# OpenMatchmaking/microservice-matchmaking

Hardware: AMD Instinct MI355X
Metric: matched players/sec over 1M-player pool (higher is better)
Workload: dtype int32

## Files before the change

include/mm_engine.h:

```cpp
#ifndef MM_ENGINE_H
#define MM_ENGINE_H

#include <stdint.h>

#ifdef __cplusplus
extern "C" {
#endif

#define MM_ABI_VERSION 1u

#define MM_MAX_GROUPS 16u
#define MM_MAX_MODES  16u
#define MM_MAX_ROLES  8u
#define MM_MAX_TEAMS  4u
#define MM_MAX_LOBBY  16u

#define MM_CONS_MODE(c)   ((uint32_t)(c) & 0xFu)
#define MM_CONS_REGION(c) (((uint32_t)(c) >> 4) & 0xFFu)
#define MM_CONS_PARTY(c)  (((uint32_t)(c) >> 12) & 0xFu)
#define MM_CONS_ROLE(c)   (((uint32_t)(c) >> 16) & 0xFu)
#define MM_CONS_MAKE(mode, region, party, role)                                          \
    (((uint32_t)(mode) & 0xFu) | (((uint32_t)(region) & 0xFFu) << 4) |                  \
     (((uint32_t)(party) & 0xFu) << 12) | (((uint32_t)(role) & 0xFu) << 16))
#define MM_CONS_USER_MASK 0x000FFFFFu
// ... 93 lines not shown
    uint32_t pair_ptimeout_us;
    uint32_t pair_pinject;
    uint32_t pair_tiles_max;
    uint32_t pair_tile_fixed;
    uint32_t pair_xcd;
    uint32_t pair_group_min;
    uint32_t pair_nxseg;
    uint32_t pair_nxstage;
    uint32_t pair_tune;
    uint32_t team_batch;
    uint32_t team_f2;
    uint32_t team_rebuild;
    uint32_t team_emit_max;
    uint32_t team_split;
    uint32_t team_fwait;
    uint32_t team_fix_max;
    uint32_t team_fix_t8;
    uint32_t team_fix_t4;
    uint32_t team_pull_xcd;
    uint32_t team_nowait;
    uint32_t team_late;
    uint32_t team_late0;
    uint32_t team_cap;
} mm_tuning;

int mm_tuning_default(mm_tuning* t);
int mm_tuning_set(mm_tuning* t, const char* name, uint32_t value);
const char* mm_tuning_name(uint32_t index);
int mm_engine_create_ex(const mm_config* cfg, const mm_tuning* tuning, mm_engine** out);
int mm_tuning_get(const mm_engine* e, mm_tuning* t);

int mm_reset(mm_engine* e);


int mm_enqueue(mm_engine* e, uint32_t n, const int32_t* rating, const uint32_t* cons,
               const uint8_t* group, uint32_t* out_slot, mm_enqueue_stats* st);

int mm_enqueue_device(mm_engine* e, uint32_t n, const int32_t* d_rating,
                      const uint32_t* d_cons, uint32_t* first_slot, mm_enqueue_stats* st);

int mm_cancel(mm_engine* e, uint32_t n, const uint32_t* slot);


int mm_tick(mm_engine* e, uint32_t mode, uint32_t* n_matches, mm_stats* stats);

int mm_matches(mm_engine* e, uint32_t first, uint32_t count, uint32_t* slots, float* score,
// ... 42 lines not shown
    uint32_t crit_round_passes;
    uint32_t crit_late_passes;
    uint32_t crit_late_lobbies;
    uint32_t degraded;
    uint32_t crit_timed_passes;
    uint32_t crit_timed_hops;
    uint32_t crit_barrier_cycles;
    uint32_t crit_hop_cycles;
    uint32_t clk_cycles;
    uint32_t clk_wall_ticks;
    uint32_t pair_nx_init_ns;
    uint32_t pair_tested_lo, pair_tested_hi;
    uint32_t pair_tested_nx_lo, pair_tested_nx_hi;
    uint32_t crit_team_group;
    uint32_t crit_team_passes;
    uint32_t crit_team_f_passes;
    uint32_t crit_team_fc_passes;
    uint32_t crit_team_late_passes;
    uint32_t crit_team_f_lobbies;
    uint32_t crit_team_fc_lobbies;
    uint32_t crit_team_late_lobbies;
    uint32_t crit_team_lookups;
    uint32_t crit_team_late_lookups;
} mm_path_stats;
int mm_path_stats_get(mm_engine* e, mm_path_stats* out);

int mm_last_hip_error(const mm_engine* e);

#ifdef __cplusplus
}
#endif
#endif
```

microservice_matchmaking_amd/_abi.py:

```python
from __future__ import annotations

import ctypes as C
import time
from dataclasses import dataclass

import numpy as np

MM_ABI_VERSION = 1
MM_MAX_GROUPS = 16
MM_MAX_MODES = 16
MM_MAX_ROLES = 8
MM_MAX_TEAMS = 4
MM_MAX_LOBBY = 16
MM_MODE_REGION_FILTER = 1
MM_MODE_PARTY_FILTER = 2
MM_CFG_TIMING = 1
MM_WAIT_HIST = 33
NO_SLOT = 0xFFFFFFFF

STATUS_NAMES = {
    0: "MM_OK", -1: "MM_ERR_INVALID_ARG", -2: "MM_ERR_NO_DEVICE", -3: "MM_ERR_OOM",
    -4: "MM_ERR_FULL", -5: "MM_ERR_HIP", -6: "MM_ERR_INTERNAL", -7: "MM_ERR_ABI",
    -8: "MM_ERR_RANGE", -9: "MM_ERR_STATE",
}
# ... 34 lines not shown


class MMEnqueueStats(C.Structure):
    _fields_ = [("accepted", C.c_uint32), ("rejected", C.c_uint32),
                ("bucket_ms", C.c_float), ("total_ms", C.c_float)]

    def as_dict(self):
        return {n: getattr(self, n) for n, _ in self._fields_}


class MMPathStats(C.Structure):
    _fields_ = [(n, C.c_uint32) for n in (
        "size", "mode", "paths", "host_looks",
        "pair_rounds_launches", "pair_rounds_passes", "pair_round_launches", "pair_tiled_passes",
        "pair_stops_timeout", "pair_stops_xcd", "pair_stops_inject", "pair_yields",
        "pair_persist_off", "pair_cooldown", "pair_stops_total",
        "team_f_launches", "team_fc_launches", "team_late_launches", "team_build_launches",
        "team_flags_late", "team_flags_late_total",
        "crit_group", "crit_passes", "crit_rounds_passes", "crit_rounds_hops", "crit_round_passes", "crit_late_passes",
        "crit_late_lobbies", "degraded",
        "crit_timed_passes", "crit_timed_hops", "crit_barrier_cycles", "crit_hop_cycles", "clk_cycles", "clk_wall_ticks",
        "pair_nx_init_ns", "pair_tested_lo", "pair_tested_hi", "pair_tested_nx_lo", "pair_tested_nx_hi",
        "crit_team_group", "crit_team_passes", "crit_team_f_passes", "crit_team_fc_passes", "crit_team_late_passes",
        "crit_team_f_lobbies", "crit_team_fc_lobbies", "crit_team_late_lobbies", "crit_team_lookups", "crit_team_late_lookups")]

    def as_dict(self):
        return {n: int(getattr(self, n)) for n, _ in self._fields_ if n != "size"}


class MMWaitGroup(C.Structure):
    _fields_ = [("waiting", C.c_uint32), ("oldest_age", C.c_uint32), ("age_sum", C.c_uint64),
                ("hist", C.c_uint32 * MM_WAIT_HIST), ("pad", C.c_uint32)]

    def as_dict(self):
        return {"waiting": int(self.waiting), "oldest_age": int(self.oldest_age), "age_sum": int(self.age_sum),
                "hist": np.asarray(self.hist[:], dtype=np.uint32)}


class MMError(RuntimeError):
    def __init__(self, status, where):
        self.status = int(status)
        super().__init__("%s failed: %s (%d)" % (where, STATUS_NAMES.get(self.status, "?"), self.status))


def cons_make(mode=0, region=0, party=0, role=0):
    mode, region, party, role = (np.asarray(x, dtype=np.uint32) for x in (mode, region, party, role))
    return ((mode & 0xF) | ((region & 0xFF) << 4) | ((party & 0xF) << 12) | ((role & 0xF) << 16)).astype(np.uint32)
# ... 416 lines not shown
```

microservice_matchmaking_amd/csrc/mm_engine.hip:

```cpp
#include <hip/hip_runtime.h>

#include <stdint.h>
#include <stdio.h>
#include <stdlib.h>
#include <string.h>
#include <time.h>

#include <dlfcn.h>

#include <algorithm>
#include <mutex>
#include <cmath>
#include <new>
#include <vector>

#include "../../include/mm_engine.h"
#include "../../include/mm_wait.h"
#include <mm_gfx950.h>


#define MM_NO_SLOT 0xFFFFFFFFu
#define MM_ST_FREE 0
#define MM_ST_LIVE 1
#define MM_ST_CANCELLED 2
// ... 904 lines not shown
    uint32_t* d_tk_chunkB;
    uint32_t* d_tk_fdone;
    uint32_t team_seq;
    uint32_t* d_tk_sqi;
    uint32_t tk_memb;
    uint32_t tk_chunk_stride;
    std::vector<uint32_t> tk_last_len;
    uint32_t dbg_last_w, dbg_last_c;
    ChainDev* h_chains;
    uint32_t* h_counters;
    std::vector<uint8_t> h_state;
    uint32_t next_slot;
    uint32_t cancel_pending;
    std::vector<uint32_t> r_released;
    uint32_t* h_rslots;
    float* h_rscore;
    uint32_t* h_rpass;
    uint32_t r_n, r_L;
    hipStream_t copy_stream;
    hipEvent_t ev_copy;
    bool ev_copy_pending;
    uint32_t r_base[MM_MAX_GROUPS], r_cnt[MM_MAX_GROUPS], r_pre[MM_MAX_GROUPS + 1];
    uint32_t r_sent[MM_MAX_GROUPS];
    uint32_t r_marked[MM_MAX_GROUPS];
    bool r_based;
    bool poisoned;
    uint32_t ticks_seen;
    bool clock_on;
    uint32_t clock_now;
    uint32_t* d_stamp;
    uint32_t* d_wt_rows;
    uint32_t wt_max_chunks;
    uint32_t* d_wt_out;
    WaitGroupDev* d_wt_stats;
    uint32_t* d_wt_matched;
    std::vector<uint32_t> x_slot, x_group, x_age;
    std::vector<uint32_t> x_new;
    std::vector<int32_t> x_rating;
    std::vector<uint32_t> x_cons, x_stamp;
    uint32_t* d_mv_cols;
    uint8_t* d_mv_group;
    uint32_t* h_mwait;
    uint32_t mw_n;
};

struct RoctxApi {
// ... 293 lines not shown
    MM_TD(pair_ptimeout_us, "MM_PAIR_PTIMEOUT_US", 5000u, 0u, 1000000u, 0u),
    MM_TD(pair_pinject, "MM_PAIR_PINJECT", 0u, 0u, 0xFFFFFFFFu, 0u),
    MM_TD(pair_tiles_max, "MM_PAIR_TILES", PK_TILES_MAX, 1u, 4096u, 0u),
    MM_TD(pair_tile_fixed, "MM_PAIR_TILE", 0u, 0u, 1u, 0u),
    MM_TD(pair_xcd, "MM_PAIR_XCD", 1u, 0u, 1u, 0u),
    MM_TD(pair_group_min, "MM_PAIR_GROUP", PK_GROUP_MIN, 0u, 0xFFFFFFFFu, 0u),
    MM_TD(pair_nxseg, "MM_PAIR_NXSEG", 0u, 64u, NXI_SEG, 1u),
    MM_TD(pair_nxstage, "MM_PAIR_NXSTAGE", 0u, 0u, 0xFFFFFFFFu, 0u),
    MM_TD(pair_tune, "MM_PAIR_TUNE", 0u, 0u, 0xFFFFFFFFu, 0u),
    MM_TD(team_batch, "MM_TEAM_BATCH", 16u, 1u, 4096u, 0u),
    MM_TD(team_f2, "MM_TEAM_F2", 32u, 0u, 0xFFFFFFFFu, 0u),
    MM_TD(team_rebuild, "MM_TEAM_REBUILD", 8u, 1u, 4096u, 0u),
    MM_TD(team_emit_max, "MM_TEAM_EMIT_MAX", TC_EMIT_MAX, 1u, TC_EMIT_MAX, 0u),
    MM_TD(team_split, "MM_TEAM_SPLIT", 1u, 0u, 1u, 0u),
    MM_TD(team_fwait, "MM_TEAM_FWAIT", 1u << 14, 0u, 0xFFFFFFFFu, 0u),
    MM_TD(team_fix_max, "MM_TEAM_FIXMAX", 0xFFFFFFFFu, 0u, 0xFFFFFFFFu, 0u),
    MM_TD(team_fix_t8, "MM_TEAM_FIXT8", 10u, 0u, 0xFFFFFFFFu, 0u),
    MM_TD(team_fix_t4, "MM_TEAM_FIXT4", 64u, 0u, 0xFFFFFFFFu, 0u),
    MM_TD(team_pull_xcd, "MM_TEAM_PULLX", 1u, 0u, 1u, 0u),
    MM_TD(team_nowait, "MM_TEAM_NOWAIT", 0u, 0u, 0xFFFFFFFFu, 0u),
    MM_TD(team_late, "MM_TEAM_LATE", 6u, 0u, 0xFFFFFFFFu, 0u),
    MM_TD(team_late0, "MM_TEAM_LATE0", 512u, 0u, 0xFFFFFFFFu, 0u),
    MM_TD(team_cap, "MM_TEAM_CAP", TT_SCAN_CAP, 1u, 4096u, 0u),
};
#undef MM_TD
static const uint32_t k_tune_n = (uint32_t)(sizeof(k_tune) / sizeof(k_tune[0]));
static_assert(sizeof(mm_tuning) == (sizeof(k_tune) / sizeof(k_tune[0]) + 1u) * sizeof(uint32_t), "every field of mm_tuning has its row in k_tune");

static bool tune_in_range(const TuneDesc& d, uint32_t v)
{
    if (d.kind == 1u) return v == 0u || (v >= d.lo && v <= d.hi && (v & (v - 1u)) == 0u);
    return v >= d.lo && v <= d.hi;
}
static uint32_t& tune_field(mm_tuning* t, const TuneDesc& d) { return *(uint32_t*)((char*)t + d.off); }

static void tune_defaults(mm_tuning* full)
{
    full->size = (uint32_t)sizeof(mm_tuning);
    for (uint32_t i = 0; i < k_tune_n; ++i) {
        const TuneDesc& d = k_tune[i];
        uint32_t v = d.def;
        const char* s = getenv(d.env);
        if (s && *s) {
            char* end = NULL;
            unsigned long long x = strtoull(s, &end, 0);
            bool ok = end && *end == 0 && end != s && x <= 0xFFFFFFFFull;
// ... 438 lines not shown
#endif
#ifndef MM_RESULTS_MIN_TEAM
#define MM_RESULTS_MIN_TEAM 4096u
#endif
static void results_set_bases(mm_engine* e, const uint32_t* before, uint32_t L)
{
    uint32_t run = 0;
    for (uint32_t g = 0; g < e->cfg.n_groups; ++g) {
        e->r_base[g] = run;
        run += before[g] / L + 1u;
    }
    e->r_based = true;
}

static void results_mark(mm_engine* e, uint32_t g, uint32_t to, uint32_t L)
{
    const uint32_t from = e->r_marked[g];
    if (to <= from) return;
    const uint32_t* const sl = e->h_rslots + (size_t)(e->r_base[g] + from) * L;
    for (size_t i = 0, n = (size_t)(to - from) * L; i < n; ++i) e->h_state[sl[i]] = MM_ST_FREE;
    e->r_marked[g] = to;
}

static int results_absorb(mm_engine* e, uint32_t L)
{
    if (!e->ev_copy_pending) return MM_OK;
    HIPCHK(e, hipEventSynchronize(e->ev_copy));
    e->ev_copy_pending = false;
    for (uint32_t g = 0; g < e->cfg.n_groups; ++g) results_mark(e, g, e->r_sent[g], L);
    return MM_OK;
}

static int results_send(mm_engine* e, const uint32_t* n_out, uint32_t L, uint32_t min_new, bool* on_main = nullptr)
{
    uint32_t fresh = 0;
    for (uint32_t g = 0; g < e->cfg.n_groups; ++g) fresh += n_out[g] > e->r_sent[g] ? n_out[g] - e->r_sent[g] : 0u;
    if (on_main) *on_main = false;
    if (fresh < min_new) return MM_OK;
    MMTRY(results_absorb(e, L));
    if (on_main != nullptr && fresh <= MM_TAIL_MAX && e->tn.results_tail) {
        TailArgs A;
        memset(&A, 0, sizeof(A));
        A.n_groups = e->cfg.n_groups; A.L = L; A.out_slot_stride = e->out_slot_stride; A.out_rec_stride = e->out_rec_stride;
        for (uint32_t g = 0; g < e->cfg.n_groups; ++g) {
            const uint32_t a = e->r_sent[g], b = n_out[g] > a ? n_out[g] : a;
            A.from[g] = a; A.base[g] = e->r_base[g]; A.pre[g + 1u] = A.pre[g] + (b - a);
            e->r_sent[g] = b;
        }
        A.total = A.pre[e->cfg.n_groups];
        if (A.total) {
            hipLaunchKernelGGL(k_results_tail, dim3((A.total + 255u) / 256u), dim3(256), 0, e->stream, A, e->d_out_slots, e->d_out_score,
                               e->d_out_pass, e->h_rslots, e->h_rscore, e->h_rpass);
            HIPCHK(e, hipGetLastError());
        }
        *on_main = true;
        return MM_OK;
    }
    const bool main_st = on_main != nullptr && fresh <= 8192u;
    hipStream_t const st = main_st ? e->stream : e->copy_stream;
    for (uint32_t g = 0; g < e->cfg.n_groups; ++g) {
        const uint32_t a = e->r_sent[g], b = n_out[g];
        if (b <= a) continue;
// ... 161 lines not shown
    {
        uint32_t seg = 256u, stage = NXI_STAGE;
        while (seg < NXI_SEG && (unsigned long long)bound > 8192ull * seg) seg <<= 1;
        if (e->tn.pair_nxseg) seg = e->tn.pair_nxseg;
        if (e->tn.pair_nxstage) stage = e->tn.pair_nxstage;
        if (stage < seg + 64u) stage = seg + 64u;
        if (stage > NXI_STAGE) stage = NXI_STAGE;
        const bool timing = (cfg.flags & MM_CFG_TIMING) != 0;
        if (timing) HIPCHK(e, hipEventRecord(e->ev_nx[0], e->stream));
        hipLaunchKernelGGL(kp_nx_init, dim3((bound + seg - 1u) / seg + 1u, G), dim3(NXI_THREADS), 0, e->stream, P, seg, stage);
        if (timing) { HIPCHK(e, hipEventRecord(e->ev_nx[1], e->stream)); e->ev_nx_set = true; }
    }
    HIPCHK(e, hipGetLastError());
    uint32_t tail_no[MM_MAX_GROUPS];
    bool tail_send = false;
    memset(e->ps_hand, 0, sizeof(e->ps_hand));
    if (bound >= PL_MAX) {
        uint32_t tiles = (bound + PK_T - 1u) / PK_T + 1u;
        if (tiles > e->pk_max_tiles) tiles = e->pk_max_tiles;
        bool after_persist = false;
        uint32_t last_tp = 0;
        uint32_t idle_looks = 0;
        unsigned long long last_progress = ~0ull;
        for (uint32_t guard = 0;; ++guard) {
            if (idle_looks > 64u) return MM_ERR_INTERNAL;
            MMTRY(look_launch(e, e->d_pchains, e->h_pchains, G * sizeof(PairChain)));
            MMTRY(look_wait(e));
            ++e->ps.host_looks;
            if (e->tn.debug && guard >= 200u && guard % 200u == 0u) {
                fprintf(stderr, "[mm-pair] look %u: cool-down %u, persist %d, last tile length %u;", guard, e->pair_pcool, (int)kp_rounds_on(e), last_tp);
                for (uint32_t g = 0; g < G; ++g) {
                    const PairChain& pc = e->h_pchains[g];
                    if (pc.fast) fprintf(stderr, " g%u[stage %u m %u qlen %u passes %u compact %u pfail 0x%x]", g, pc.stage, pc.m, pc.qlen, pc.passes, pc.want_compact, pc.pfail);
                }
                fprintf(stderr, "\n");
            }
            {
                unsigned long long progress = 0;
                for (uint32_t g = 0; g < G; ++g) {
                    const PairChain& pc = e->h_pchains[g];
                    if (pc.fast) progress += (unsigned long long)pc.passes + ((unsigned long long)pc.m << 32) + (pc.stage == PS_TILED ? 1u : 0u) + pc.want_compact;
                }
                idle_looks = progress == last_progress ? idle_looks + 1u : 0u;
                last_progress = progress;
            }
            bool tiled = false, compact = false;
            uint32_t longest = 0;
            for (uint32_t g = 0; g < G; ++g) {
                const PairChain& pc = e->h_pchains[g];
                P.bm[g] = 0;
// ... 71 lines not shown
                for (uint32_t cand = PK_TMAX / 4u; cand < PK_TMAX; cand <<= 1)
                    if ((longest + cand - 1u) / cand <= tiles_max) { tp = cand; break; }
            if (last_tp && tp > last_tp && !compact) {
                hipLaunchKernelGGL(kp_ask_compact, dim3(G), dim3(64), 0, e->stream, P, 0xFFFFFFFFu);
                compact = true;
                last_tp = 0;
            }
            tiles = (longest + tp - 1u) / tp;
#define TILE_LAUNCH(KERNEL, GRID, BLOCK, ...)                                                                              \
    do {                                                                                                                   \
        if (tp == PK_TMAX) hipLaunchKernelGGL(KERNEL<PK_TMAX>, GRID, BLOCK, 0, e->stream, __VA_ARGS__);                    \
        else if (tp == PK_TMAX / 2u) hipLaunchKernelGGL(KERNEL<PK_TMAX / 2u>, GRID, BLOCK, 0, e->stream, __VA_ARGS__);     \
        else hipLaunchKernelGGL(KERNEL<PK_TMAX / 4u>, GRID, BLOCK, 0, e->stream, __VA_ARGS__);                             \
    } while (0)
#define COMPACT_LAUNCH()                                                                                                   \
    do {                                                                                                                   \
        TILE_LAUNCH(kc_words, dim3(tiles, G), dim3(256), P);                                                               \
        TILE_LAUNCH(kc_plan, dim3(G), dim3(1024), P);                                                                      \
        TILE_LAUNCH(kc_scatter, dim3(tiles, G), dim3(1024), P);                                                            \
        TILE_LAUNCH(kc_commit, dim3(G), dim3(1024), P);                                                                    \
    } while (0)
            if (compact) {
                COMPACT_LAUNCH();
                HIPCHK(e, hipGetLastError());
                continue;
            }
            last_tp = tp;
            for (uint32_t g = 0; g < G; ++g) P.pyq[g] = 0;
            P.pyq[yield_g] = yield_q;
            {
                P.grp = (e->tn.pair_group_min && tiles >= e->tn.pair_group_min && tp == PK_TMAX) ? PK_GS : 0u;
                const uint32_t ngr = P.grp ? (tiles + P.grp - 1u) / P.grp : 0u;
                dim3 rgrid(tiles, G);
                P.xslots = 0;
                uint32_t tof[MM_MAX_GROUPS];
                for (uint32_t g = 0; g < G; ++g) tof[g] = P.bm[g] ? (P.bm[g] + tp - 1u) / tp : 0u;
                if (persist) {
                    const uint32_t slots = pair_xcd_map(P, tof, G, true);
                    if (slots) {
                        P.grp = 0;
                        const uint32_t K = e->tn.pair_pbatch, slice = MM_PERSIST_SLICE ? MM_PERSIST_SLICE : K + 1u;
                        for (uint32_t it = 0; it <= K; it += slice)
                            TILE_LAUNCH(kp_rounds, dim3(8u * slots), dim3(PT_THREADS), P, it, it + slice < K + 1u ? it + slice : K + 1u, K);
                        ++e->ps.pair_rounds_launches;
                        after_persist = true;
                        COMPACT_LAUNCH();
                        HIPCHK(e, hipGetLastError());
                        MMTRY(results_absorb(e, M.L));
                        MMTRY(results_send(e, sent_no, M.L, e->tn.results_early ? MM_RESULTS_MIN_PAIR : 0xFFFFFFFFu));
                        continue;
                    }
                    P.xslots = 0;
                }
                if (e->tn.pair_xcd) {
                    const uint32_t slots = pair_xcd_map(P, tof, G);
                    if (slots) rgrid = dim3(8u * slots);
                }
                uint32_t r = e->round_ctr;
                TILE_LAUNCH(kp_round, rgrid, dim3(PT_THREADS), P, r, 1u);
                ++r;
                if (P.grp) TILE_LAUNCH(kp_group, dim3(ngr, G), dim3(1024), P, r);
                for (uint32_t b = 0; b < (want_fit && e->tn.pair_batch > 12u ? 12u : e->tn.pair_batch); ++b) {
                    TILE_LAUNCH(kp_round, rgrid, dim3(PT_THREADS), P, r, 0u);
                    ++e->ps.pair_round_launches;
                    ++r;
                    if (P.grp) TILE_LAUNCH(kp_group, dim3(ngr, G), dim3(1024), P, r);
                }
                TILE_LAUNCH(kp_round_commit, dim3(tiles, G), dim3(256), P, r);
                hipLaunchKernelGGL(kp_round_stage, dim3(G), dim3(64), 0, e->stream, P, r);
                COMPACT_LAUNCH();
                e->round_ctr = r;
            }
#undef COMPACT_LAUNCH
#undef TILE_LAUNCH
            HIPCHK(e, hipGetLastError());
            MMTRY(results_absorb(e, M.L));
            MMTRY(results_send(e, sent_no, M.L, e->tn.results_early ? MM_RESULTS_MIN_PAIR : 0xFFFFFFFFu));
        }
    }
    hipLaunchKernelGGL(kp_late, dim3(G), dim3(PL_THREADS), 0, e->stream, P);
    hipLaunchKernelGGL(kp_finish, dim3(G), dim3(1024), 0, e->stream, P);
    HIPCHK(e, hipGetLastError());
    if (tail_send) {
        MMTRY(results_absorb(e, M.L));
        MMTRY(results_send(e, tail_no, M.L, e->tn.results_early ? MM_RESULTS_MIN_PAIR : 0xFFFFFFFFu));
    }
    return MM_OK;
}

static void report_team(const mm_engine* e)
{
    const uint32_t G = e->cfg.n_groups;
    for (uint32_t g = 0; g < G; ++g) {
        const TeamChain& t = e->h_tchains[g];
        const uint32_t np = t.passes + 1u;
        fprintf(stderr, "[mm-team] g%u fast %u m %u passes %u out %u left %u | cancel tick: head sat out %u, seated %u, lobby filtered %u, anchor moved %u x | "
                "kt_f, the middle chunk, cycles per pass: first loads %u, probes + lists %u, replacements %u, look-ups from scratch %u, barrier %u, step C %u; anchors at work per pass %u | "
                "F values written %u, changed after the first pass %u | kt_chase: sub-queue entries looked at by the stored lobby's fills %u, by %u look-ups %u\n",
                g, t.fast, t.m, t.passes, t.n_out, t.qlen,
                t.dbg[6] & 1u, (t.dbg[6] >> 1) & 1u, (t.dbg[6] >> 2) & 1u, t.dbg[7],
// ... 363 lines not shown
    return rc;
}

static int tick_impl(mm_engine* e, uint32_t mode, uint32_t* n_matches, mm_stats* stats)
{
    RoctxRange rr_tick("mm_tick");
    const double t0 = host_now_ms();
    const mm_config& cfg = e->cfg;
    const uint32_t G = cfg.n_groups;
    const ModeDev M = make_mode_dev(cfg.modes[mode]);
    const bool timing = (cfg.flags & MM_CFG_TIMING) != 0;
    const bool purge = e->cancel_pending > 0;
    e->r_n = 0;
    e->mw_n = 0;
    e->r_L = M.L;
    {
        const uint32_t tot = e->ps.team_flags_late_total;
        memset(&e->ps, 0, sizeof(e->ps));
        e->ps.mode = mode;
        e->ps.team_flags_late_total = tot;
    }
    if (e->ev_copy_pending) { (void)hipEventSynchronize(e->ev_copy); e->ev_copy_pending = false; }
    e->r_based = false;
    for (uint32_t g = 0; g < G; ++g) { e->r_sent[g] = 0; e->r_marked[g] = 0; e->r_cnt[g] = 0; }

    HIPCHK(e, hipMemsetAsync(e->d_counters, 0, sizeof(uint32_t), e->stream));
    if (timing) HIPCHK(e, hipEventRecord(e->ev[0], e->stream));
    if (purge) {
        hipLaunchKernelGGL(k_purge, dim3(G), dim3(WK_THREADS), 0, e->stream, mode, G, cfg.capacity, e->d_chains,
                           e->d_q_rating, e->d_q_cons, e->d_q_slot, e->d_state, e->d_released, e->d_counters);
        HIPCHK(e, hipGetLastError());
    }
    if (timing) HIPCHK(e, hipEventRecord(e->ev[1], e->stream));
    const bool use_pair = M.team_size == 1u && M.teams == 2u && !e->tn.force_generic;
    if (use_pair) {
        RoctxRange rr("mm_tick/pair walk");
        e->ps.paths |= MM_PATH_PAIR;
        MMTRY(pair_walk(e, mode, M, purge));
    }
    bool team_any = false;
    if (!use_pair && !e->tn.force_generic && e->live_upper >= TT_MIN) {
        RoctxRange rr("mm_tick/team walk");
        MMTRY(team_walk(e, mode, M, purge, &team_any));
        if (team_any) e->ps.paths |= MM_PATH_TEAM;
    }
    if (!e->ps.paths) e->ps.paths = MM_PATH_GENERIC;
    WalkParams P;
// ... 855 lines not shown
```

microservice_matchmaking_amd/csrc/mm_pair.inc:

```

#define PK_NO 0xFFFFFFFFu
#define PK_ABORT 0xFFFFFFFEu

#define NX_INV 0u
#define NX_NONE 0xFFFFu
#define NX_FAR 0xFFFEu

#ifndef PK_T
#define PK_T 8192u
#endif
enum : uint32_t { PK_TMAX = PK_T };
#undef PK_T
static constexpr uint32_t PK_T = PK_TMAX;
#ifndef PK_TILES_MAX
#define PK_TILES_MAX 40u
#endif
#define PK_XSEG 4u
#ifndef PK_GS
#define PK_GS 8u
#endif
#ifndef PK_GROUP_MIN
#define PK_GROUP_MIN 64u
#endif
#ifndef PL_MAX
// ... 63 lines not shown
    uint32_t rounds;
    uint32_t ghops;
    uint32_t gtry, gstale;
    uint32_t tm[16];
    uint32_t pfail;
    uint32_t ppass;
    uint32_t pxm;
    uint32_t pslow[4];
    uint32_t ptm[16];
    RoundState rs[2];
};

struct PairParams {
    uint32_t mode, n_groups, capacity, window, eqmask;
    uint32_t out_slot_stride, out_rec_stride, bits_stride;
    uint32_t pstride;
    uint32_t tune;
    uint32_t purge;
    uint8_t* state;
    uint32_t* released;
    uint32_t* n_released;
    ChainDev* chains;
    PairChain* pchains;
    int32_t* q_rating;
    uint32_t* q_cons;
    uint32_t* q_slot;
    uint32_t* key[2];
    uint32_t* oidx[2];
    uint16_t* nx16[2];
    uint32_t* bits[2];
    uint32_t* scratch;
    uint16_t* g16;
    uint32_t* rec2[2];
    uint16_t* exa[2];
    uint32_t* bitsp[2];
    uint32_t* headp[2];
    uint4* grec;
    uint32_t grp;
    uint32_t xslots;
    uint32_t xseg[8][PK_XSEG];
    uint16_t xcnt[8][PK_XSEG];
    uint32_t gstride;
    unsigned long long* pbar;
    uint32_t* pxmask;
    uint32_t ptimeout0, ptimeout1;
    uint32_t pinject;
// ... 1684 lines not shown
#undef EMIT_STORE
#undef SEAT_PATCH
}

#define PF_TIMEOUT 1u
#define PF_XCD 2u
#define PF_INJECT 3u
#define PF_YIELD 4u

template <uint32_t TP>
struct RoundsRes {
    alignas(16) uint32_t key[2 * TP + 64];
    alignas(16) uint16_t nx[TP];
    alignas(16) uint16_t g[TP + 8];
    alignas(16) uint32_t pc[TP + 64];
    alignas(16) uint32_t bits[2 * TP / 32 + 4];
    uint32_t cnt[16];
    uint16_t nw[TP / 32 + 2];
    uint16_t path[TP / 2 + 72];
    RoundState S, N;
    uint32_t my[8];
    uint32_t ctl[4];
    uint32_t tm[16];
};

static __device__ __forceinline__ uint32_t w_scan_fit_x(const uint32_t* key, const uint32_t* bits, uint32_t akey, uint32_t from, uint32_t m,
                                                        uint32_t w, int lane)
{
    uint32_t klo, krng;
    pk_bounds(akey, w, klo, krng);
    for (uint32_t p = from; p < m; p += 256u) {
        uint32_t bw[4], kv[4];
#pragma unroll
        for (uint32_t u = 0; u < 4u; ++u) {
            const uint32_t c = p + 64u * u + (uint32_t)lane;
            bw[u] = c < m ? xld(bits + (c >> 5)) : 0u;
            kv[u] = c < m ? key[c] : 0xFFFFFFFFu;
        }
#pragma unroll
        for (uint32_t u = 0; u < 4u; ++u) {
            const uint32_t c = p + 64u * u + (uint32_t)lane;
            const unsigned long long b = __ballot(((bw[u] >> (c & 31u)) & 1u) != 0u && pk_in(kv[u], klo, krng));
            if (b) return p + 64u * u + (uint32_t)__ffsll(b) - 1u;
        }
    }
    return PK_NO;
// ... 29 lines not shown
                t = ((sg >> 8) & 0xFFu) + sl * (sg >> 16);
                found = true;
            }
            if (!found) sl -= c;
        }
        if (!found) return;
    }
    PairChain* const pc = P.pchains + g;
    const uint32_t m = P.bm[g], buf = P.bbuf[g];
    if (m == 0u || t >= (m + PK_T - 1u) / PK_T) return;
    const int tid_o = threadIdx.x;
    const uint32_t w = P.window, ntiles = (m + PK_T - 1u) / PK_T;
    const uint32_t c = P.mode * P.n_groups + g;
    const size_t qo = (size_t)c * P.capacity, po = (size_t)g * P.pstride;
    const uint32_t base = t * PK_T;
    const uint32_t tl = dev_min_u32(PK_T, m - base);
    const uint32_t hl = dev_min_u32(2u * PK_T, m - base);
    const uint32_t* const key = P.key[buf] + po;
    const uint32_t* const oidx = P.oidx[buf] + po;
    uint16_t* const gnx = P.nx16[buf] + po + base;
    uint32_t* const bits_com = P.bits[buf] + (size_t)g * P.bits_stride;
    const uint32_t own_words = (tl + 31u) >> 5, hwords = (hl + 31u) >> 5;
    unsigned long long* const bar = P.pbar + g;
    long long tq = clock64();
#define TMARK(K_) do { if (tmr) { const long long now = clock64(); L.tm[K_] += (uint32_t)(now - tq); tq = now; } } while (0)

    if (it_begin == 0u) {
        const int tid = tid_o;
        MM_RESIDENT_FRESH(L);
        if (tid == 0) {
            RoundState S;
            S.live = 1; S.done = 0; S.want_compact = 0; S.rounds = pc->rounds;
            S.qlen = pc->qlen; S.passes = pc->passes; S.n_out = pc->n_out; S.has_anchor = pc->has_anchor;
            S.a_key = pc->a_key; S.a_slot = pc->a_slot; S.a_cons = pc->a_cons; S.a_team = pc->a_team;
            S.a_rating = pc->a_rating; S.pairs = pc->pairs; S.scanned = pc->scanned;
            S.pos0 = pc->pos0; S.changed0 = pc->changed0; S.extra0 = pc->extra0; S.a_oi = PK_NO;
            L.S = S;
            L.N = S;
            L.ctl[0] = 0; L.ctl[1] = 0; L.ctl[2] = 0;
            for (int k = 0; k < 16; ++k) L.tm[k] = 0;
        }
        for (uint32_t i = tid; i < 2u * PK_T / 32u + 4u; i += PT_THREADS) s_bits[i] = i < hwords ? bits_com[(base >> 5) + i] : 0u;
        copy_words_x4((uint32_t*)s_nx, (const uint32_t*)gnx, (tl + 1u) >> 1, tid, PT_THREADS);
        if (tid < 8) s_g[PK_T + tid] = (uint16_t)PK_T;
        if (tid == 0) { s_cnt[1] = 0; s_cnt[2] = 0; s_cnt[3] = 0; s_cnt[4] = 0; }
        if ((uint32_t)tid < RP_MAXLONG) s_pc[RP_MAXLONG + tid] = PK_NO;
        __syncthreads();
        prep_stage_keys<PK_T>(s_key, s_bits, key + base, hl, tid);
        __syncthreads();
    } else if (L.ctl[0]) return;

    uint32_t stop = 0;
    bool ended = false;
    uint32_t tst = 0;
    long long dw0 = 0;
    uint32_t dwork = 0, dn = 0;
    for (uint32_t it = it_begin; it < it_end; ++it) {
        int tid_l = tid_o;
        TW_LAUNDER(tid_l);
        const int tid = tid_l, lane = tid & 63, wave = tid >> 6;
        const bool tmr = t == 1u && tid == 0;
        const uint32_t cpar = it & 1u, npar = cpar ^ 1u;
        const uint32_t* const bits_src = P.bitsp[cpar] + (size_t)g * P.bits_stride;
        uint32_t* const bits_dst = P.bitsp[npar] + (size_t)g * P.bits_stride;
        uint32_t em_off = PK_NO, em_ia = 0, em_iq = 0, em_score = 0, hd_off = PK_NO, hd_iq = 0, hd_score = 0;
        uint32_t em_sa = 0, em_sq = 0, hd_sq = 0, hd_sa = 0, hd_team = 0, em_pass = 0;
        bool em_loaded = false;
#define EMIT_LOAD() do { if (!em_loaded) { em_loaded = true;                                                   \
        if (em_off != PK_NO) { em_sa = P.q_slot[qo + em_ia]; em_sq = P.q_slot[qo + em_iq]; }                  \
        if (hd_off != PK_NO) hd_sq = P.q_slot[qo + hd_iq]; } } while (0)
#define EMIT_STORE() do { EMIT_LOAD();                                                                         \
        uint32_t* const eos = P.out_slots + (size_t)g * P.out_slot_stride;                                    \
        if (em_off != PK_NO) {                                                                                \
            eos[2u * em_off] = em_sa; eos[2u * em_off + 1u] = em_sq;                                          \
            P.out_score[(size_t)g * P.out_rec_stride + em_off] = (float)(int32_t)em_score;                    \
            P.out_pass[(size_t)g * P.out_rec_stride + em_off] = em_pass; }                                    \
        if (hd_off != PK_NO) {                                                                                \
            eos[2u * hd_off + hd_team] = hd_sa; eos[2u * hd_off + (1u - hd_team)] = hd_sq;                    \
            P.out_score[(size_t)g * P.out_rec_stride + hd_off] = (float)(int32_t)hd_score;                    \
// ... 13 lines not shown
                    if ((wv & 0xFFFFFFFFull) >= need) break;
                    if (f == 0u && xld(P.pyield) != 0u) {
                        const unsigned long long nv = wv | ((unsigned long long)(PF_YIELD | (it << 8)) << 32);
                        if (atomicCAS(bar, wv, nv) == wv) { verdict = PF_YIELD | (it << 8); break; }
                        continue;
                    }
                    if (f == 0u && wall_clock64() - t0 > limit) {
                        const unsigned long long nv = wv | ((unsigned long long)(PF_TIMEOUT | (it << 8)) << 32);
                        if (atomicCAS(bar, wv, nv) == wv) { verdict = PF_TIMEOUT | (it << 8); break; }
                        continue;
                    }
                    __builtin_amdgcn_s_sleep(1);
                }
                if (!verdict && it == 1u) {
                    const uint32_t xm = xld(P.pxmask + g);
                    if (xm & (xm - 1u)) verdict = PF_XCD | (1u << 8);
                }
                L.ctl[1] = verdict;
            }
            __syncthreads();
            tw_sinv();
            if (L.ctl[1]) { stop = L.ctl[1]; break; }
            TMARK(0);
            if (tid == 0 && (P.tune & 0x10000u)) dw0 = clock64();
            const RoundState S = L.S;
            em_pass = S.passes;
            if (wave != 0) {
                for (uint32_t i = PK_T / 32u + (uint32_t)tid - 64u; i < hwords; i += PT_THREADS - 64u) {
                    const uint32_t nw_ = xld(bits_src + (base >> 5) + i);
                    uint32_t gone = s_bits[i] & ~nw_;
                    s_bits[i] = nw_;
                    while (gone) {
                        const uint32_t b = (uint32_t)__ffs((int)gone) - 1u;
                        gone &= gone - 1u;
                        s_key[(i << 5) + b] |= PK_DEAD;
                    }
                }
                if ((uint32_t)tid - 64u < RP_MAXLONG) s_pc[RP_MAXLONG + tid - 64] = PK_NO;
                __builtin_amdgcn_fence(__ATOMIC_RELEASE, "workgroup");
                wave_lockstep();
                if (lane == 0) atomicAdd(&s_cnt[4], 1u);
                while (lds_ld(&s_cnt[4]) < (uint32_t)(PT_THREADS / 64 - 1)) __builtin_amdgcn_s_sleep(1);
                __builtin_amdgcn_fence(__ATOMIC_ACQUIRE, "workgroup");
                if (it != K && !(P.tune & 0x4000u))
                    repair_sweep<PK_T>(s_key, s_nx, s_pc, &s_cnt[1], s_pc + 2u * RP_MAXLONG + (uint32_t)wave * RP_TODO, bits_src + (base >> 5),
                                       tl, hl, base + hl == m, w, lane, (uint32_t)wave - 1u, PT_THREADS / 64u - 1u, tst);
            }
// ... 213 lines not shown
            }
            __syncthreads();
            TMARK(9);
        }
        struct { uint32_t live, has_anchor, a_key; } N;
        N.live = L.S.live; N.has_anchor = L.S.has_anchor; N.a_key = L.S.a_key;
        if (!N.live || it == K) { EMIT_STORE(); ended = true; break; }
        if (it > 0u && L.S.qlen <= P.pyq[g]) {
            if (t == 0u && tid == 0) __hip_atomic_store(P.pyield, 1u, __ATOMIC_RELAXED, __HIP_MEMORY_SCOPE_AGENT);
            EMIT_STORE(); ended = true; break;
        }

        for (uint32_t i = tid; i < own_words; i += PT_THREADS) bits_dst[(base >> 5) + i] = s_bits[i];
        if (tid == 0) { s_cnt[0] = PK_NO; s_cnt[4] = 0; }
        prep_repair<PK_T>(s_key, s_nx, s_pc, &s_cnt[1], bits_src + (base >> 5), tl, hl, base + hl == m, w, tid, tst,
                          tmr ? L.tm : nullptr);
        EMIT_LOAD();
        if (N.has_anchor) {
            uint32_t klo, krng;
            pk_bounds(N.a_key, w, klo, krng);
            uint32_t best = PK_NO;
            for (uint32_t i = tid; i < tl; i += PT_THREADS)
                if (best == PK_NO && pk_in(s_key[i], klo, krng)) best = i;
            const unsigned long long b = __ballot(best != PK_NO);
            if (b) {
                uint32_t v = best;
                for (int dd = 1; dd < 64; dd <<= 1) { const uint32_t o2 = (uint32_t)__shfl((int)v, lane ^ dd); v = o2 < v ? o2 : v; }
                if (lane == 0) atomicMin(&s_cnt[0], v);
            }
        }
        prep_tables<PK_T>(s_key, s_nx, s_bits, s_nw, s_pc, s_g, P.rec2[npar] + po + base, P.exa[npar] + po + base,
                          nullptr, tl, tid, tmr ? L.tm : nullptr);
        if (tmr) tq = clock64();
        if (tid == 0) P.headp[npar][(size_t)g * P.max_tiles + t] = s_cnt[0] == PK_NO ? PK_NO : base + s_cnt[0];
        {
            uint32_t acc = 0;
            const uint32_t* const rb = P.rec2[npar] + po + base;
            for (uint32_t i = (uint32_t)tid * 16u; i < tl; i += PT_THREADS * 16u) acc ^= xld(rb + i);
            for (uint32_t i = (uint32_t)tid * 16u; i < own_words; i += PT_THREADS * 16u) acc ^= xld(bits_dst + (base >> 5) + i);
            TW_SINK(acc);
        }
        tw_store_wait();
        __syncthreads();
        if (tid == 0) {
            unsigned long long add = 1ull;
            if (it == 0u) {
                const uint32_t o = atomicOr(P.pxmask + g, 1u << mm_xcc_id());
                TW_KEEP(o);
                tw_store_wait();
            }
            if (it > 0u && (P.tune & 0x10000u)) { dwork += (uint32_t)(clock64() - dw0); ++dn; }
            if (P.pinject && P.pinject == it && t == 1u) {
                for (;;) {
                    const unsigned long long o = xld64(bar);
                    if (o >> 32) { atomicAdd(bar, 1ull); break; }
                    if (atomicCAS(bar, o, (o + 1ull) | ((unsigned long long)(PF_INJECT | ((it + 1u) << 8)) << 32)) == o) break;
                }
            } else atomicAdd(bar, add);
        }
        EMIT_STORE();
        TMARK(4);
    }
#undef EMIT_LOAD
#undef EMIT_STORE
    if (!ended && !stop) return;

    const int tid = tid_o, lane = tid & 63;
    const bool tmr = t == 1u && tid == 0;
    __syncthreads();
    for (uint32_t i = tid; i < own_words; i += PT_THREADS) bits_com[(base >> 5) + i] = s_bits[i];
    for (uint32_t i = tid; i < tl; i += PT_THREADS)
        if (s_nx[i] == NX_PEND) s_nx[i] = (uint16_t)NX_INV;
    __syncthreads();
    {
// ... 1 lines not shown
        for (uint32_t i = tid; i < (tl + 7u) >> 3; i += PT_THREADS) nx4[i] = ((const uint4*)s_nx)[i];
    }
    if (tid == 0) L.ctl[0] = 1;
    if (t == 0 && tid == 0) {
        const RoundState S = L.S;
        pc->qlen = S.qlen; pc->passes = S.passes; pc->n_out = S.n_out; pc->has_anchor = S.has_anchor;
        pc->a_key = S.a_key; pc->a_team = S.a_team;
        if (S.has_anchor && S.a_oi != PK_NO) {
            pc->a_slot = P.q_slot[qo + S.a_oi]; pc->a_rating = P.q_rating[qo + S.a_oi]; pc->a_cons = P.q_cons[qo + S.a_oi];
        } else { pc->a_slot = S.a_slot; pc->a_rating = S.a_rating; pc->a_cons = S.a_cons; }
        pc->pairs = S.pairs; pc->scanned = S.scanned; pc->rounds = S.rounds;
        pc->want_compact = S.want_compact | ((!S.done && P.pyq[g] && S.qlen <= P.pyq[g]) ? 1u : 0u);
        pc->pos0 = S.pos0; pc->changed0 = S.changed0; pc->extra0 = S.extra0;
        if (S.done) pc->stage = PS_DONE;
        pc->pfail = stop;
        pc->ppass += L.ctl[2];
        pc->pxm = xld(P.pxmask + g);
    }
    if (tmr) {
        for (int k = 0; k < 16; ++k) if (L.tm[k]) atomicAdd(&pc->ptm[k], L.tm[k]);
        atomicAdd(&pc->ptm[5], L.ctl[2]);
    }
    if ((P.tune & 0x2000u) && lane == 0 && tst) atomicAdd(&pc->tested, (unsigned long long)tst);
    if ((P.tune & 0x10000u) && tid == 0 && dn) {
        uint32_t* const dg = (uint32_t*)(P.grec + (size_t)g * P.gstride + t);
        atomicAdd(dg + 0, dwork);
        atomicAdd(dg + 1, dn);
    }
#undef TMARK
}

template <uint32_t TP>
__global__ __launch_bounds__(1024) void kp_group(PairParams P, uint32_t r_next)
{
    constexpr uint32_t PK_T = TP;
    (void)PK_T;
    const uint32_t g = blockIdx.y, gr = blockIdx.x;
    const uint32_t m = P.bm[g];
    if (m == 0u) return;
    const uint32_t ntiles = (m + PK_T - 1u) / PK_T;
    if (gr * P.grp >= ntiles) return;
    const uint32_t cpar = r_next & 1u;
    if (!(P.pchains + g)->rs[cpar].live) return;
    const size_t po = (size_t)g * P.pstride;
    const uint32_t* const rec = P.rec2[cpar] + po;
    const uint32_t* const bits = P.bitsp[cpar] + (size_t)g * P.bits_stride;
    uint4* const out = P.grec + (size_t)g * P.gstride + (size_t)gr * PK_T;
    const uint32_t t0 = gr * P.grp, gend = t0 + P.grp;
    __shared__ uint32_t s_mark[PK_T / 32u];
    __shared__ uint32_t s_list[PK_T];
// ... 187 lines not shown
        const uint32_t o = P.nx16[buf][po + i];
        uint32_t no = NX_INV;
        if (o == NX_NONE) no = NX_NONE;
        else if (o != NX_INV && o != NX_FAR) {
            const uint32_t q = i + o;
            const uint32_t qw = q < m ? bits[q >> 5] : 0u;
            if ((qw >> (q & 31u)) & 1u) {
                const uint32_t rq = tbase[q / PK_T] + wpre[q >> 5] + (uint32_t)__popc(qw & ((1u << (q & 31u)) - 1u));
                no = rq - r;
            }
        }
        P.nx16[buf ^ 1u][po + r] = (uint16_t)no;
    }
}

template <uint32_t TP>
__global__ __launch_bounds__(1024) void kc_commit(PairParams P)
{
    constexpr uint32_t PK_T = TP;
    (void)PK_T;
    const uint32_t g = blockIdx.x;
    PairChain* const pc = P.pchains + g;
    if (threadIdx.x == 0) { P.pbar[g] = 0ull; P.pxmask[g] = 0u; if (g == 0u) *P.pyield = 0u; }
    if (!pc->fast || pc->stage != PS_TILED || !pc->want_compact) return;
    const int tid = threadIdx.x;
    const uint32_t nm = pc->new_m;
    const uint32_t nt = (nm + PK_T - 1u) / PK_T;
    uint32_t* const talive = tc_row(P, TC_ALIVE, g);
    for (uint32_t t = tid; t < P.max_tiles; t += 1024) talive[t] = t < nt ? dev_min_u32(PK_T, nm - t * PK_T) : 0u;
    __syncthreads();
    if (tid == 0) {
        pc->m = nm;
        pc->ntiles = nt;
        pc->buf ^= 1u;
        pc->want_compact = 0;
        if (nm < PL_MAX) pc->stage = PS_LATE;
    }
}

__global__ __launch_bounds__(1024) void kp_finish(PairParams P)
{
    __shared__ uint32_t wtot[16];
    const int tid = threadIdx.x, lane = tid & 63, wave = tid >> 6;
    const uint32_t g = blockIdx.x;
    PairChain* const pc = P.pchains + g;
    if (!pc->fast) return;
    const uint32_t c = P.mode * P.n_groups + g;
    ChainDev* const ch = P.chains + c;
    const size_t qo = (size_t)c * P.capacity, po = (size_t)g * P.pstride;
    const uint32_t m = pc->m;
    const uint32_t* const oidx = P.oidx[pc->buf] + po;
    const uint32_t* const bits = P.bits[pc->buf] + (size_t)g * P.bits_stride;
    uint32_t* const t_rating = P.key[pc->buf ^ 1u] + po;
    uint32_t* const t_cons = P.oidx[pc->buf ^ 1u] + po;
    uint32_t* const t_slot = P.scratch + po;
    uint32_t wr = 0;
    for (uint32_t base = 0; base < m; base += 1024u) {
        const uint32_t i = base + (uint32_t)tid;
        const bool live = i < m && ((bits[i >> 5] >> (i & 31u)) & 1u);
        const unsigned long long bm = __ballot(live);
// ... 45 lines not shown
```

Baseline: 107.3 million.

## Publish pair-chain state from commit kernel and slice result absorption between looks

The commit kernel now writes each group's PairChain state directly into host-mapped memory, so the host can wait on the stream instead of launching a separate look copy and waiting on it. Result absorption is split into an arrival step and a sliced marking step that stops as soon as the GPU stream goes idle, so host-side bookkeeping overlaps kernel execution. The tiled kernel's timer and debug counters move from registers into shared state, and the wave-min reduction now uses ballot-based bit search instead of shuffles. The cost is more complex host/device ordering and extra zero-copy host writes from every commit block.

```diff
diff --git a/include/mm_engine.h b/include/mm_engine.h
--- a/include/mm_engine.h
+++ b/include/mm_engine.h
@@ -139,6 +139,8 @@
     uint32_t team_late;
     uint32_t team_late0;
     uint32_t team_cap;
+    uint32_t look_commit;
+    uint32_t absorb_slices;
 } mm_tuning;
 
 int mm_tuning_default(mm_tuning* t);
@@ -227,6 +229,9 @@
     uint32_t crit_team_late_lobbies;
     uint32_t crit_team_lookups;
     uint32_t crit_team_late_lookups;
+    uint32_t results_early_sends;
+    uint32_t looks_commit;
+    uint32_t absorb_deferred;
 } mm_path_stats;
 int mm_path_stats_get(mm_engine* e, mm_path_stats* out);
 
diff --git a/microservice_matchmaking_amd/_abi.py b/microservice_matchmaking_amd/_abi.py
--- a/microservice_matchmaking_amd/_abi.py
+++ b/microservice_matchmaking_amd/_abi.py
@@ -80,7 +80,8 @@
         "crit_timed_passes", "crit_timed_hops", "crit_barrier_cycles", "crit_hop_cycles", "clk_cycles", "clk_wall_ticks",
         "pair_nx_init_ns", "pair_tested_lo", "pair_tested_hi", "pair_tested_nx_lo", "pair_tested_nx_hi",
         "crit_team_group", "crit_team_passes", "crit_team_f_passes", "crit_team_fc_passes", "crit_team_late_passes",
-        "crit_team_f_lobbies", "crit_team_fc_lobbies", "crit_team_late_lobbies", "crit_team_lookups", "crit_team_late_lookups")]
+        "crit_team_f_lobbies", "crit_team_fc_lobbies", "crit_team_late_lobbies", "crit_team_lookups", "crit_team_late_lookups",
+        "results_early_sends", "looks_commit", "absorb_deferred")]
 
     def as_dict(self):
         return {n: int(getattr(self, n)) for n, _ in self._fields_ if n != "size"}
diff --git a/microservice_matchmaking_amd/csrc/mm_engine.hip b/microservice_matchmaking_amd/csrc/mm_engine.hip
--- a/microservice_matchmaking_amd/csrc/mm_engine.hip
+++ b/microservice_matchmaking_amd/csrc/mm_engine.hip
@@ -950,6 +950,7 @@
     bool ev_copy_pending;
     uint32_t r_base[MM_MAX_GROUPS], r_cnt[MM_MAX_GROUPS], r_pre[MM_MAX_GROUPS + 1];
     uint32_t r_sent[MM_MAX_GROUPS];
+    uint32_t r_here[MM_MAX_GROUPS];
     uint32_t r_marked[MM_MAX_GROUPS];
     bool r_based;
     bool poisoned;
@@ -1289,6 +1290,8 @@
     MM_TD(team_late, "MM_TEAM_LATE", 6u, 0u, 0xFFFFFFFFu, 0u),
     MM_TD(team_late0, "MM_TEAM_LATE0", 512u, 0u, 0xFFFFFFFFu, 0u),
     MM_TD(team_cap, "MM_TEAM_CAP", TT_SCAN_CAP, 1u, 4096u, 0u),
+    MM_TD(look_commit, "MM_LOOK_COMMIT", 1u, 0u, 1u, 0u),
+    MM_TD(absorb_slices, "MM_ABSORB_SLICES", 1u, 0u, 1u, 0u),
 };
 #undef MM_TD
 static const uint32_t k_tune_n = (uint32_t)(sizeof(k_tune) / sizeof(k_tune[0]));
@@ -1773,12 +1776,30 @@
     e->r_marked[g] = to;
 }
 
-static int results_absorb(mm_engine* e, uint32_t L)
+static int results_arrive(mm_engine* e)
 {
     if (!e->ev_copy_pending) return MM_OK;
     HIPCHK(e, hipEventSynchronize(e->ev_copy));
     e->ev_copy_pending = false;
-    for (uint32_t g = 0; g < e->cfg.n_groups; ++g) results_mark(e, g, e->r_sent[g], L);
+    for (uint32_t g = 0; g < e->cfg.n_groups; ++g) e->r_here[g] = e->r_sent[g];
+    return MM_OK;
+}
+
+#define MM_ABSORB_SLICE 4096u
+
+static int results_absorb(mm_engine* e, uint32_t L, bool all = true)
+{
+    MMTRY(results_arrive(e));
+    for (uint32_t g = 0; g < e->cfg.n_groups; ++g) {
+        if (all) { results_mark(e, g, e->r_here[g], L); continue; }
+        while (e->r_marked[g] < e->r_here[g]) {
+            const hipError_t q = hipStreamQuery(e->stream);
+            if (q == hipSuccess) { ++e->ps.absorb_deferred; return MM_OK; }
+            if (q != hipErrorNotReady) { e->last_hip = (int)q; return MM_ERR_HIP; }
+            const uint32_t step = MM_ABSORB_SLICE / L + 1u, left = e->r_here[g] - e->r_marked[g];
+            results_mark(e, g, e->r_marked[g] + (left < step ? left : step), L);
+        }
+    }
     return MM_OK;
 }
 
@@ -1788,7 +1809,8 @@
     for (uint32_t g = 0; g < e->cfg.n_groups; ++g) fresh += n_out[g] > e->r_sent[g] ? n_out[g] - e->r_sent[g] : 0u;
     if (on_main) *on_main = false;
     if (fresh < min_new) return MM_OK;
-    MMTRY(results_absorb(e, L));
+    if (e->tn.absorb_slices) MMTRY(results_arrive(e));
+    else MMTRY(results_absorb(e, L));
     if (on_main != nullptr && fresh <= MM_TAIL_MAX && e->tn.results_tail) {
         TailArgs A;
         memset(&A, 0, sizeof(A));
@@ -1996,10 +2018,38 @@
         uint32_t last_tp = 0;
         uint32_t idle_looks = 0;
         unsigned long long last_progress = ~0ull;
+        bool look_by_commit = false, look_queued = false;
+        P.hlook = e->tn.look_commit ? e->h_pchains : nullptr;
+        const auto batch_launched = [&](bool send, const uint32_t* sent_no) -> int {
+            HIPCHK(e, hipGetLastError());
+            look_by_commit = P.hlook != nullptr;
+            if (!e->tn.absorb_slices) {
+                if (!send) return MM_OK;
+                MMTRY(results_absorb(e, M.L));
+                return results_send(e, sent_no, M.L, e->tn.results_early ? MM_RESULTS_MIN_PAIR : 0xFFFFFFFFu);
+            }
+            if (!look_by_commit) { MMTRY(look_launch(e, e->d_pchains, e->h_pchains, G * sizeof(PairChain))); look_queued = true; }
+            if (send) MMTRY(results_send(e, sent_no, M.L, e->tn.results_early ? MM_RESULTS_MIN_PAIR : 0xFFFFFFFFu));
+            return results_absorb(e, M.L, false);
+        };
+        const auto batch_done = [&](bool send, const uint32_t* sent_no) -> int {
+            uint32_t had = 0, has = 0;
+            for (uint32_t g = 0; g < G; ++g) had += e->r_sent[g];
+            const int rc = batch_launched(send, sent_no);
+            for (uint32_t g = 0; g < G; ++g) has += e->r_sent[g];
+            if (rc == MM_OK && has != had) ++e->ps.results_early_sends;
+            return rc;
+        };
         for (uint32_t guard = 0;; ++guard) {
             if (idle_looks > 64u) return MM_ERR_INTERNAL;
-            MMTRY(look_launch(e, e->d_pchains, e->h_pchains, G * sizeof(PairChain)));
-            MMTRY(look_wait(e));
+            if (look_by_commit) {
+                HIPCHK(e, hipStreamSynchronize(e->stream));
+                ++e->ps.looks_commit;
+            } else {
+                if (!look_queued) MMTRY(look_launch(e, e->d_pchains, e->h_pchains, G * sizeof(PairChain)));
+                MMTRY(look_wait(e));
+            }
+            look_by_commit = look_queued = false;
             ++e->ps.host_looks;
             if (e->tn.debug && guard >= 200u && guard % 200u == 0u) {
                 fprintf(stderr, "[mm-pair] look %u: cool-down %u, persist %d, last tile length %u;", guard, e->pair_pcool, (int)kp_rounds_on(e), last_tp);
@@ -2117,7 +2167,7 @@
     } while (0)
             if (compact) {
                 COMPACT_LAUNCH();
-                HIPCHK(e, hipGetLastError());
+                MMTRY(batch_done(false, nullptr));
                 continue;
             }
             last_tp = tp;
@@ -2140,9 +2190,7 @@
                         ++e->ps.pair_rounds_launches;
                         after_persist = true;
                         COMPACT_LAUNCH();
-                        HIPCHK(e, hipGetLastError());
-                        MMTRY(results_absorb(e, M.L));
-                        MMTRY(results_send(e, sent_no, M.L, e->tn.results_early ? MM_RESULTS_MIN_PAIR : 0xFFFFFFFFu));
+                        MMTRY(batch_done(true, sent_no));
                         continue;
                     }
                     P.xslots = 0;
@@ -2168,9 +2216,7 @@
             }
 #undef COMPACT_LAUNCH
 #undef TILE_LAUNCH
-            HIPCHK(e, hipGetLastError());
-            MMTRY(results_absorb(e, M.L));
-            MMTRY(results_send(e, sent_no, M.L, e->tn.results_early ? MM_RESULTS_MIN_PAIR : 0xFFFFFFFFu));
+            MMTRY(batch_done(true, sent_no));
         }
     }
     hipLaunchKernelGGL(kp_late, dim3(G), dim3(PL_THREADS), 0, e->stream, P);
@@ -2580,7 +2626,7 @@
     }
     if (e->ev_copy_pending) { (void)hipEventSynchronize(e->ev_copy); e->ev_copy_pending = false; }
     e->r_based = false;
-    for (uint32_t g = 0; g < G; ++g) { e->r_sent[g] = 0; e->r_marked[g] = 0; e->r_cnt[g] = 0; }
+    for (uint32_t g = 0; g < G; ++g) { e->r_sent[g] = 0; e->r_here[g] = 0; e->r_marked[g] = 0; e->r_cnt[g] = 0; }
 
     HIPCHK(e, hipMemsetAsync(e->d_counters, 0, sizeof(uint32_t), e->stream));
     if (timing) HIPCHK(e, hipEventRecord(e->ev[0], e->stream));
diff --git a/microservice_matchmaking_amd/csrc/mm_pair.inc b/microservice_matchmaking_amd/csrc/mm_pair.inc
--- a/microservice_matchmaking_amd/csrc/mm_pair.inc
+++ b/microservice_matchmaking_amd/csrc/mm_pair.inc
@@ -109,6 +109,7 @@
     uint32_t* n_released;
     ChainDev* chains;
     PairChain* pchains;
+    PairChain* hlook;
     int32_t* q_rating;
     uint32_t* q_cons;
     uint32_t* q_slot;
@@ -1839,6 +1840,8 @@
     uint32_t my[8];
     uint32_t ctl[4];
     uint32_t tm[16];
+    uint32_t tq;
+    uint32_t dw[3];
 };
 
 static __device__ __forceinline__ uint32_t w_scan_fit_x(const uint32_t* key, const uint32_t* bits, uint32_t akey, uint32_t from, uint32_t m,
@@ -1914,8 +1917,7 @@
     uint32_t* const bits_com = P.bits[buf] + (size_t)g * P.bits_stride;
     const uint32_t own_words = (tl + 31u) >> 5, hwords = (hl + 31u) >> 5;
     unsigned long long* const bar = P.pbar + g;
-    long long tq = clock64();
-#define TMARK(K_) do { if (tmr) { const long long now = clock64(); L.tm[K_] += (uint32_t)(now - tq); tq = now; } } while (0)
+#define TMARK(K_) do { if (tmr) { const uint32_t now = (uint32_t)clock64(); L.tm[K_] += now - L.tq; L.tq = now; } } while (0)
 
     if (it_begin == 0u) {
         const int tid = tid_o;
@@ -1931,6 +1933,8 @@
             L.N = S;
             L.ctl[0] = 0; L.ctl[1] = 0; L.ctl[2] = 0;
             for (int k = 0; k < 16; ++k) L.tm[k] = 0;
+            L.tq = (uint32_t)clock64();
+            L.dw[0] = 0; L.dw[1] = 0; L.dw[2] = 0;
         }
         for (uint32_t i = tid; i < 2u * PK_T / 32u + 4u; i += PT_THREADS) s_bits[i] = i < hwords ? bits_com[(base >> 5) + i] : 0u;
         copy_words_x4((uint32_t*)s_nx, (const uint32_t*)gnx, (tl + 1u) >> 1, tid, PT_THREADS);
@@ -1945,8 +1949,6 @@
     uint32_t stop = 0;
     bool ended = false;
     uint32_t tst = 0;
-    long long dw0 = 0;
-    uint32_t dwork = 0, dn = 0;
     for (uint32_t it = it_begin; it < it_end; ++it) {
         int tid_l = tid_o;
         TW_LAUNDER(tid_l);
@@ -2006,7 +2008,7 @@
             tw_sinv();
             if (L.ctl[1]) { stop = L.ctl[1]; break; }
             TMARK(0);
-            if (tid == 0 && (P.tune & 0x10000u)) dw0 = clock64();
+            if (tid == 0 && (P.tune & 0x10000u)) L.dw[0] = (uint32_t)clock64();
             const RoundState S = L.S;
             em_pass = S.passes;
             if (wave != 0) {
@@ -2266,16 +2268,21 @@
             uint32_t best = PK_NO;
             for (uint32_t i = tid; i < tl; i += PT_THREADS)
                 if (best == PK_NO && pk_in(s_key[i], klo, krng)) best = i;
-            const unsigned long long b = __ballot(best != PK_NO);
+            unsigned long long b = __ballot(best != PK_NO);
             if (b) {
-                uint32_t v = best;
-                for (int dd = 1; dd < 64; dd <<= 1) { const uint32_t o2 = (uint32_t)__shfl((int)v, lane ^ dd); v = o2 < v ? o2 : v; }
+                uint32_t v = 0;
+#pragma unroll
+                for (int bit = 31 - __builtin_clz(PK_T - 1u); bit >= 0; --bit) {
+                    const unsigned long long z = __ballot(best != PK_NO && !((best >> bit) & 1u)) & b;
+                    if (z) b = z;
+                    else v |= 1u << bit;
+                }
                 if (lane == 0) atomicMin(&s_cnt[0], v);
             }
         }
         prep_tables<PK_T>(s_key, s_nx, s_bits, s_nw, s_pc, s_g, P.rec2[npar] + po + base, P.exa[npar] + po + base,
                           nullptr, tl, tid, tmr ? L.tm : nullptr);
-        if (tmr) tq = clock64();
+        if (tmr) L.tq = (uint32_t)clock64();
         if (tid == 0) P.headp[npar][(size_t)g * P.max_tiles + t] = s_cnt[0] == PK_NO ? PK_NO : base + s_cnt[0];
         {
             uint32_t acc = 0;
@@ -2293,7 +2300,7 @@
                 TW_KEEP(o);
                 tw_store_wait();
             }
-            if (it > 0u && (P.tune & 0x10000u)) { dwork += (uint32_t)(clock64() - dw0); ++dn; }
+            if (it > 0u && (P.tune & 0x10000u)) { L.dw[1] += (uint32_t)clock64() - L.dw[0]; ++L.dw[2]; }
             if (P.pinject && P.pinject == it && t == 1u) {
                 for (;;) {
                     const unsigned long long o = xld64(bar);
@@ -2341,10 +2348,10 @@
         atomicAdd(&pc->ptm[5], L.ctl[2]);
     }
     if ((P.tune & 0x2000u) && lane == 0 && tst) atomicAdd(&pc->tested, (unsigned long long)tst);
-    if ((P.tune & 0x10000u) && tid == 0 && dn) {
+    if ((P.tune & 0x10000u) && tid == 0 && L.dw[2]) {
         uint32_t* const dg = (uint32_t*)(P.grec + (size_t)g * P.gstride + t);
-        atomicAdd(dg + 0, dwork);
-        atomicAdd(dg + 1, dn);
+        atomicAdd(dg + 0, L.dw[1]);
+        atomicAdd(dg + 1, L.dw[2]);
     }
 #undef TMARK
 }
@@ -2578,20 +2585,28 @@
     const uint32_t g = blockIdx.x;
     PairChain* const pc = P.pchains + g;
     if (threadIdx.x == 0) { P.pbar[g] = 0ull; P.pxmask[g] = 0u; if (g == 0u) *P.pyield = 0u; }
-    if (!pc->fast || pc->stage != PS_TILED || !pc->want_compact) return;
     const int tid = threadIdx.x;
-    const uint32_t nm = pc->new_m;
-    const uint32_t nt = (nm + PK_T - 1u) / PK_T;
-    uint32_t* const talive = tc_row(P, TC_ALIVE, g);
-    for (uint32_t t = tid; t < P.max_tiles; t += 1024) talive[t] = t < nt ? dev_min_u32(PK_T, nm - t * PK_T) : 0u;
+    if (pc->fast && pc->stage == PS_TILED && pc->want_compact) {
+        const uint32_t nm = pc->new_m;
+        const uint32_t nt = (nm + PK_T - 1u) / PK_T;
+        uint32_t* const talive = tc_row(P, TC_ALIVE, g);
+        for (uint32_t t = tid; t < P.max_tiles; t += 1024) talive[t] = t < nt ? dev_min_u32(PK_T, nm - t * PK_T) : 0u;
+        __syncthreads();
+        if (tid == 0) {
+            pc->m = nm;
+            pc->ntiles = nt;
+            pc->buf ^= 1u;
+            pc->want_compact = 0;
+            if (nm < PL_MAX) pc->stage = PS_LATE;
+        }
+    }
+    if (P.hlook == nullptr) return;
+    __builtin_amdgcn_fence(__ATOMIC_RELEASE, "agent");
     __syncthreads();
-    if (tid == 0) {
-        pc->m = nm;
-        pc->ntiles = nt;
-        pc->buf ^= 1u;
-        pc->want_compact = 0;
-        if (nm < PL_MAX) pc->stage = PS_LATE;
-    }
+    const uint32_t* const src = (const uint32_t*)pc;
+    uint32_t* const dst = (uint32_t*)(P.hlook + g);
+    for (uint32_t i = tid; i < (uint32_t)(sizeof(PairChain) / 4u); i += 1024)
+        dst[i] = __hip_atomic_load(src + i, __ATOMIC_RELAXED, __HIP_MEMORY_SCOPE_AGENT);
 }
 
 __global__ __launch_bounds__(1024) void kp_finish(PairParams P)
```

Result: slower. 105.4 million (-1.8%).
